# gallilmaimon/DISSC

Hardware: AMD Instinct MI355X
Metric: audio-sec/sec (RTF) HiFi-GAN resynth, 10s x32 batch (higher is better)
Workload: dtype f32

## Files before the change

dissc_amd/_lib.py:

```python
import ctypes
import os

import torch

_HERE = os.path.dirname(os.path.abspath(__file__))
_LIB_NAME = "libdissc_hip.so"


def library_path():
    return os.environ.get("DISSC_HIP_LIB") or os.path.join(_HERE, _LIB_NAME)


class DisscError(RuntimeError):
    pass


class DisscTensor(ctypes.Structure):
    _fields_ = [("name", ctypes.c_char_p), ("data", ctypes.c_void_p),
                ("shape", ctypes.c_int64 * 4), ("ndim", ctypes.c_int32)]


MAX_UPS, MAX_RK = 8, 4


class DisscGenConfig(ctypes.Structure):
    _fields_ = [("model_in_dim", ctypes.c_int32), ("upsample_initial_channel", ctypes.c_int32),
                ("num_upsamples", ctypes.c_int32), ("upsample_rates", ctypes.c_int32 * MAX_UPS),
                ("upsample_kernel_sizes", ctypes.c_int32 * MAX_UPS), ("num_kernels", ctypes.c_int32),
                ("resblock_kernel_sizes", ctypes.c_int32 * MAX_RK),
                ("resblock_dilations", (ctypes.c_int32 * 3) * MAX_RK),
                ("num_embeddings", ctypes.c_int32), ("embedding_dim", ctypes.c_int32),
                ("num_speakers", ctypes.c_int32), ("has_f0", ctypes.c_int32), ("has_spkr", ctypes.c_int32)]


class DisscConvLaunch(ctypes.Structure):
    _fields_ = [(n, ctypes.c_int32) for n in ("family", "cfg", "bm", "bn", "rows", "p0", "np", "ntap", "pad_left")]


class DisscBf3Info(ctypes.Structure):
    _fields_ = [(n, ctypes.c_int32) for n in ("bm", "bn", "small_grid", "tile", "cols", "h4", "pad")]


class DisscWino8Plan(ctypes.Structure):
    _fields_ = [(n, ctypes.c_int32) for n in ("mi", "ni", "wps", "r", "ns", "unit", "ot", "cpr", "gx", "gy")]


class DisscWinoPlan(ctypes.Structure):
    _fields_ = [(n, ctypes.c_int32) for n in ("ns", "dilation", "cpr", "rh", "tw", "shv", "unit", "ot", "gx", "gy", "wgs", "lds_bytes")]


def _load():
    path = library_path()
    if not os.path.exists(path):
        raise DisscError(
            f"{path} not found: build the HIP library first "
            "(python -c 'import __graft_entry__ as g; g.build()').  "
            "dissc_amd has no CPU fallback.")
    L = ctypes.CDLL(path)
    vp, i32, i64p = ctypes.c_void_p, ctypes.c_int, ctypes.c_void_p
    L.dissc_last_error.restype = ctypes.c_char_p
    L.dissc_abi_version.restype = i32
    L.dissc_device_count.restype = i32
    L.dissc_device_name.argtypes = [i32, ctypes.c_char_p, ctypes.c_size_t]
    L.dissc_gen_create.argtypes = [ctypes.POINTER(DisscGenConfig), ctypes.POINTER(DisscTensor),
                                   ctypes.c_size_t, ctypes.POINTER(vp)]
    L.dissc_gen_create_ex.argtypes = [ctypes.POINTER(DisscGenConfig), ctypes.POINTER(DisscTensor),
                                      ctypes.c_size_t, i32, ctypes.POINTER(vp)]
    L.dissc_gen_destroy.argtypes = [vp]
    L.dissc_gen_destroy.restype = None
    L.dissc_gen_hop.argtypes = [vp]
    L.dissc_gen_workspace_bytes.argtypes = [vp, i32, i32]
    L.dissc_gen_workspace_bytes.restype = ctypes.c_size_t
    L.dissc_gen_flops.argtypes = [vp, ctypes.c_int64]
    L.dissc_gen_flops.restype = ctypes.c_double
    L.dissc_gen_flops_executed.argtypes = [vp, ctypes.c_int64]
    L.dissc_gen_flops_executed.restype = ctypes.c_double
    L.dissc_gen_forward.argtypes = [vp, i64p, vp, i64p, vp, i32, i32, vp, vp, ctypes.c_size_t, vp]
# ... 136 lines not shown
```

dissc_amd/csrc/common.h:

```cpp
#pragma once
#include <hip/hip_runtime.h>
#include <stdint.h>
#include <stdio.h>

#include <atomic>
#include <functional>
#include <mutex>
#include <string>
#include <vector>

#include "../../include/dissc_hip.h"

#ifndef DISSC_EXPERIMENTAL
#define DISSC_EXPERIMENTAL 0
#endif

namespace dissc {

void set_error(const char* fmt, ...);

#define DISSC_OPTION_LIST_DEFAULT(X) \
  X(multistream, 1, "multistream") \
  X(pair_dma, 1, "pair_dma") \
  X(precision, 0, "precision") \
  X(enc_precision, 0, "enc_precision") \
  X(use_mfma32, 1, "mfma32") \
  X(ragged_enum, 1, "ragged_enum") \
  X(lin128, 1, "lin128") \
  X(conv2s128, 1, "conv2s128") \
  X(xcd_order, 11, "xcd_order") \
  X(xcd_mg, 0, "xcd_mg") \
  X(small_grid, 1, "small_grid") \
  X(kernel_dbg, 0, "kernel_dbg") \
  X(wino_sv, 1, "wino_sv") \
  X(wino8_c64_wide, 3, "wino8_c64_wide") \
  X(wino8_mask, 0450770550, "wino8_mask") \
  X(wino8_r4_mask, 0770770010, "wino8_r4_mask") \
  X(wino8_r4, 1, "wino8_r4") \
  X(wino8, 1, "wino8") \
  X(wino, 1, "wino") \
  X(hubert_split, 1, "hubert_split") \
  X(pair_max_c, 32, "pair_max_c") \
  X(pair_f23, 3, "pair_f23") \
  X(pair_tc6, 3, "pair_tc6") \
  X(pair_f23_c64, 1, "pair_f23_c64") \
  X(pair_tc6_c64, 1, "pair_tc6_c64")
#define DISSC_OPTION_LIST_EXPERIMENTAL(X) \
  X(graphs, 0, "graphs") \
  X(graph_frames, 2048, "graph_frames") \
  X(enc_tc, 0, "enc_tc") \
  X(s2tc_xmode, 0, "s2tc_xmode") \
  X(pair_wino, 0, "pair_wino") \
  X(pairw_chv, 2, "pairw_chv")
#if DISSC_EXPERIMENTAL
#define DISSC_OPTION_LIST(X) DISSC_OPTION_LIST_DEFAULT(X) DISSC_OPTION_LIST_EXPERIMENTAL(X)
#else
#define DISSC_OPTION_LIST(X) DISSC_OPTION_LIST_DEFAULT(X)
#endif
struct Options {
#define DISSC_OPT_FIELD(f, d, k) int f = d;
  DISSC_OPTION_LIST(DISSC_OPT_FIELD)
#undef DISSC_OPT_FIELD
#if !DISSC_EXPERIMENTAL
#define DISSC_OPT_CONST(f, d, k) static constexpr int f = d;
  DISSC_OPTION_LIST_EXPERIMENTAL(DISSC_OPT_CONST)
#undef DISSC_OPT_CONST
#endif
  int cfg_for_bm[5] = {6, 5, 7, 1, 0};
  int cfg32_for_bm[4] = {3, 2, 1, 0};
// ... 163 lines not shown
int conv32_cfg_bn(int cfg);
void conv32_set_cfg(int bm_class, int cfg);
void pack_conv_weights32(const float* w, int Cout, int Cin, int KS, std::vector<float>& packed,
                         int& Mpad, int& nchunk, int groups);
void pack_conv_weights_bf3(const float* w, int Cout, int Cin, int KS, std::vector<float>& packed,
                           int& Mpad, int& nchunk);
int launch_conv_bf3(const ConvArgs& a, int B, int Lmax_out, hipStream_t stream);
int conv_bf3_tile_bn(int M);
struct ConvBf3Plan { int tile, BM, BN, small; };
int conv_bf3_plan(int M, int KS, int dil, int groups, int B, int Lmax_out, ConvBf3Plan& p);
bool enc_bf3_supported(int Cout, int Cin, int KS, int dil, int groups, int stride, int pad_left);
int launch_enc_bf3(const ConvArgs& a, int B, int Lmax_out, int stride, hipStream_t stream);

void pack_conv_weights(const float* w, int Cout, int Cin, int KS, std::vector<float>& packed,
                       int& Mpad, int& nchunk, int groups = 1);
void convT_phase_weights(const float* w, int Cin, int Cout, int k, int s, int p0, int np, int dlo,
                         int ntap, std::vector<float>& wc);

struct DevConv {
  float* wpack = nullptr;
  float* wpack2 = nullptr;
  float* bias = nullptr;
  float* scale = nullptr;
  float* shift = nullptr;
  int CIN = 0, M = 0, KS = 0, dil = 1, nchunk = 0, up = 1;
  int groups = 1, Mpad = 0, stride = 1, pad_left = -1;
  int up_np = 1, up_p0 = 0;
  int act = 0;
  int m32 = 0;
  int prec = 0;
  double macs_per_t = 0;
  int wino = 0;
  int wr = 3;
};
struct Batch {
  const int32_t* lengths = nullptr;
  int len_default = 0, len_mul = 1, B = 0, Lmax = 0;
  const int32_t* lengths_out = nullptr;
  int olen_default = -1;
};
inline Batch batch_of(const int32_t* lengths, int len_mul, int B, int Lmax) {
  Batch bt;
  bt.lengths = lengths; bt.len_default = bt.Lmax = Lmax; bt.len_mul = len_mul; bt.B = B;
  return bt;
}
struct EpiSpec {
  int epi = EPI_STORE;
  const float* res = nullptr;
  float* acc = nullptr;
  float mrf_div = 1.f, out_slope = 0.f;
};
inline EpiSpec epi_of(int epi, const float* res = nullptr, float* acc = nullptr, float mrf_div = 1.f) {
  EpiSpec ep;
  ep.epi = epi; ep.res = res; ep.acc = acc; ep.mrf_div = mrf_div;
  return ep;
}
int upload(const std::vector<float>& h, float** d);
int pack_thread_count();
int run_pack_tasks(const std::vector<std::function<int()>>& tasks, int nthr, const Options& opt, int prec);
int conv_m32_rule(int Mg, int groups);
void conv_geometry(DevConv& dc, int Cout, int Cin, int KS, int dil, int groups, int stride, int pad_left);
struct ConvTGroup { int p0, np, dlo, ntap; };
void convT_groups(int Cout, int k, int s, std::vector<ConvTGroup>& out);
int conv_launch_cfg32(const DevConv& dc, int B, int Lmax_out);
int conv_launch_info(const DevConv& dc, int B, int Lmax_out, int* family, int* cfg, int* bm, int* bn);
int make_conv(const float* w, const float* bias, int Cout, int Cin, int KS, int dil, DevConv& dc,
              int groups = 1, int stride = 1, int pad_left = -1);
int make_convT(const float* w, const float* bias, int Cin, int Cout, int k, int s,
               std::vector<DevConv>& groups);
int set_affine(DevConv& dc, const float* scale, const float* shift, int n);
void free_conv(DevConv& dc);
int run_conv(const DevConv& dc, const float* x, float* out, const Batch& bt, const EpiSpec& ep, int C_x, int ldx, int ldo,
             float slope, hipStream_t stream, int dma_in = 0);

bool wino_supported(int Cout, int Cin, int KS, int dil);
int make_wino(const float* w, const float* bias, int C, int KS, int dil, DevConv& dc);
double wino_executed_macs_per_t(int C, int KS);
int run_wino(const DevConv& dc, const float* x, float* out, const Batch& bt, const EpiSpec& ep, int ldx, int ldo, float slope,
             hipStream_t stream);
struct WinoPlan { int inst, NS, dil, CPR, RH, TW, SHV, unit, OT, gx, gy, wgs, lds_bytes; };
int wino_plan(int C, int KS, int dil, int B, int Lmax, WinoPlan& p);

bool wino8_supported(int Cout, int Cin, int KS, int dil);
bool wino8_r4_supported(int C, int KS, int dil);
int make_wino8(const float* w, const float* bias, int C, int KS, int dil, DevConv& dc, int R = 3);
double wino8_executed_macs_per_t(int C, int KS, int R);
int run_wino8(const DevConv& dc, const float* x, float* out, const Batch& bt, const EpiSpec& ep, int ldx, int ldo, float slope,
              hipStream_t stream);
struct Wino8Plan { int inst, R, NS, MI, NI, WPS, unit, OT, CPR, gx, gy; };
int wino8_plan(int C, int KS, int dil, int R, int B, int Lmax, Wino8Plan& p);

struct DevPairW {
  float* w1 = nullptr;
  float* w2 = nullptr;
  float* b1 = nullptr;
  float* b2 = nullptr;
  int C = 0, KS = 0, dil = 1;
  int form = 0;
};
bool pair_f23_supported(int C, int KS, int dil);
bool pair_tc6_supported(int C, int KS, int dil);
bool pairw43_built();
int pack_pairw43(const float* w, int C, int KS, float** dev);
int launch_pairw43(const DevPairW& pw, const float* x, float* out, const Batch& bt, const EpiSpec& ep, int ld, float slope,
                   hipStream_t stream);
bool pairw_supported(int C, int KS, int dil);
bool pair_form_supported(int form, int C, int KS, int dil);
int pair_reg_tile(int form, int C, int KS, int dil);
int make_pairw(const float* w1, const float* b1, const float* w2, const float* b2, int C, int KS, int dil, int form, DevPairW& pw);
void free_pairw(DevPairW& pw);
int launch_respair_wino(const DevPairW& pw, const float* x, float* out, const Batch& bt, const EpiSpec& ep, int ld, float slope,
                        hipStream_t stream);

bool respair_supported(int C, int KS, int dil);
int launch_respair(const DevConv& c1, const DevConv& c2, const float* x, float* out, const Batch& bt, const EpiSpec& ep, int ld,
                   float slope, hipStream_t stream);

bool resblock_bf3_supported(int C, int KS, const int* dil);
void pack_resblock_bf3(int C, int KS, const float* const* w6, std::vector<float>& packed);
struct Bf3Block { int C, KS; const int* dil; const float *wpack, *bias; };
int launch_resblock_bf3(const Bf3Block& blk, const float* x, const Batch& bt, const EpiSpec& ep, int ld, float slope, int m0, int m1,
                        hipStream_t stream);
// ... 30 lines not shown
```

dissc_amd/csrc/conv_wino8.hip:

```cpp
#include <string.h>

#include <type_traits>

#include "common.h"
#include "conv_epilogue32.h"
#include "wino_common.h"

namespace dissc {


struct Wino8Args {
  const float* x;
  const float* wpack;
  const float* bias;
  const float* res;
  float* out;
  float* acc;
  const int32_t* lengths;
  int len_default, len_mul;
  int C, nchunk, pad;
  int ldx, ldo;
  long long x_bstride, o_bstride;
  float slope, mrf_div;
  int epi;
  int dbg;
  int gx, gy, B;
};

static const double kW8Pt[7] = {0.0, 1.0, -1.0, 2.0, -2.0, 0.5, -0.5};
static const double kW8Scale[7] = {-1.0, -2.0 / 9.0, -2.0 / 9.0, 1.0 / 90.0, 1.0 / 90.0, 32.0 / 45.0, 32.0 / 45.0};
static double w8_g(int p, int i, int R) {
  if (p == 7) return i == R - 1 ? 1.0 : 0.0;
  double v = kW8Scale[p];
  for (int e = 0; e < i; ++e) v *= kW8Pt[p];
  return v;
}

template <int P>
__device__ __forceinline__ float w8_bt(float r0, float r1, float r2, float r3, float r4, float r5, float r6, float r7) {
  if constexpr (P == 0) return fmaf(5.25f, r2 - r4, r6 - r0);
  if constexpr (P == 1) return fmaf(-4.25f, r3 + r4, (r1 + r2) + (r5 + r6));
  if constexpr (P == 2) return fmaf(4.25f, r3 - r4, (r2 - r1) + (r6 - r5));
  if constexpr (P == 3) return fmaf(0.5f, r1, fmaf(0.25f, r2, fmaf(-2.5f, r3, fmaf(-1.25f, r4, fmaf(2.f, r5, r6)))));
  if constexpr (P == 4) return fmaf(-0.5f, r1, fmaf(0.25f, r2, fmaf(2.5f, r3, fmaf(-1.25f, r4, fmaf(-2.f, r5, r6)))));
  if constexpr (P == 5) return fmaf(2.f, r1, fmaf(4.f, r2, fmaf(-2.5f, r3, fmaf(-5.f, r4, fmaf(0.5f, r5, r6)))));
  if constexpr (P == 6) return fmaf(-2.f, r1, fmaf(4.f, r2, fmaf(2.5f, r3, fmaf(-5.f, r4, fmaf(-0.5f, r5, r6)))));
  if constexpr (P == 7) return fmaf(5.25f, r3 - r5, r7 - r1);
  return 0.f;
}

constexpr int w8_rup(int n, int m) { return (n + m - 1) / m * m; }

constexpr int w8_row_len(int D, int NTU, int need, int MO) {
// ... 53 lines not shown
template <int NS, int DIL, int MI, int NI, int WPS = 2, int R = 3>
__global__ void __launch_bounds__(512, (NI == 1 ? 2 : WPS)) conv_wino8_kernel(const Wino8Args a) {
  using G = Wino8Geo<NS, DIL, MI, NI, WPS, R>;
  constexpr bool LAT = G::LAT;
  constexpr int NTH = G::NTH, D = G::D, W = G::W, NCOL = G::NCOL, OT = G::OT, NV = G::NV, RL = G::RL, MO = G::MO,
                CHF = G::CHF, CPR = G::CPR, XV = G::XV, YS = G::YS, OFF = G::OFF, RPP = G::RPP, CG = G::CG;
  extern __shared__ __attribute__((aligned(16))) float lds[];
  float* const vbuf = lds + G::WIN_FLOATS;

  const int per = 8 / a.gy;
  const int xcd = blockIdx.x & 7, kq = blockIdx.x >> 3;
  const int mt = xcd / per;
  const int lin = (xcd - mt * per) + per * kq;
  if (lin >= a.gx * a.B) return;
  const int tid = threadIdx.x;
  const int lane = tid & 63;
  int b, len = a.len_default, t0;
  if (a.lengths == nullptr) {
    b = lin / a.gx;
    t0 = (lin - b * a.gx) * OT;
    if (t0 >= len) return;
  } else {
    int tile;
    if (!ragged_tile<OT>(lin, a.B, [&](int i) { return a.lengths[i] * a.len_mul; }, b, tile, len)) return;
    t0 = tile * OT;
  }
  const int p = __builtin_amdgcn_readfirstlane(tid >> 6);
  const int l31 = lane & 31, h = lane >> 5;
  const int o = t0 - a.pad;
  const int tb = o & ~3;
  const int sh = o - tb;
  const float slope = a.slope;
  const float* xb = a.x + (size_t)b * a.x_bstride;
  const int nround = a.C / CPR;

  const int r0 = tid / NV, v0 = tid - r0 * NV;
  constexpr int dr = NTH / NV, dv = NTH - dr * NV;
  constexpr int SV = (CPR * NV + NTH - 1) / NTH;
  f32x4 sv[SV];
  auto stage_load = [&](int rd) __attribute__((always_inline)) {
    int r = r0, v = v0;
#pragma unroll
    for (int i = 0; i < SV; ++i) {
      int ci = rd * CPR + (r < CPR ? r : CPR - 1);
      ci = ci < a.C ? ci : a.C - 1;
      int t = tb + 4 * v;
      t = t < 0 ? 0 : (t > a.ldx - 4 ? a.ldx - 4 : t);
      sv[i] = *reinterpret_cast<const f32x4*>(xb + (size_t)ci * a.ldx + t);
      v += dv;
      r += dr;
      if (v >= NV) { v -= NV; ++r; }
    }
  };
  auto stage_store = [&](float* raw) __attribute__((always_inline)) {
    int r = r0, v = v0;
#pragma unroll
    for (int i = 0; i < SV; ++i) {
      if (r < CPR) {
        const int t = tb + 4 * v;
        const f32x4 val = sv[i];
        float* rowp = raw + r * CHF;
#pragma unroll
        for (int e = 0; e < 4; ++e) {
          const bool ok = (t + e) >= 0 && (t + e) < len;
          const int xs = 4 * v + e - sh + OFF * D;
          rowp[(xs % D) * RL + xs / D] = ok ? lrelu(val[e], slope) : 0.f;
        }
// ... 59 lines not shown
  int voff[NI];
#pragma unroll
  for (int ni = 0; ni < NI; ++ni) {
    int col = ni * 32 + l31;
    col = col < NCOL ? col : NCOL - 1;
    voff[ni] = (col / D) * W + (col % D) + h * XV;
  }
  f32x16 acc[MI][NI];
#pragma unroll
  for (int mi = 0; mi < MI; ++mi)
#pragma unroll
    for (int ni = 0; ni < NI; ++ni)
#pragma unroll
      for (int e = 0; e < 16; ++e) acc[mi][ni][e] = 0.f;

  const int nsub = a.C / 32;
  const int nblk = a.nchunk * NS * 2;
  f32x4 av[MI], avn[MI];
#ifndef DISSC_WINO8_BUF
#define DISSC_WINO8_BUF 1
#endif
#if DISSC_WINO8_BUF
  const __amdgpu_buffer_rsrc_t wrs = wave_rsrc(reinterpret_cast<const f32x4*>(a.wpack) + ((size_t)p * nsub + mt * MI) * nblk * 64,
                                               (unsigned)(MI * nblk) * 1024u);
  const unsigned lane16 = lane * 16u;
  auto a_load = [&](int mi, int bl) __attribute__((always_inline)) { return rsrc_load16(wrs, lane16, (unsigned)(mi * nblk + bl) * 1024u); };
#else
  const f32x4* wp[MI];
#pragma unroll
  for (int mi = 0; mi < MI; ++mi)
    wp[mi] = reinterpret_cast<const f32x4*>(a.wpack) + ((size_t)p * nsub + mt * MI + mi) * nblk * 64 + lane;
  auto a_load = [&](int mi, int bl) __attribute__((always_inline)) { return wp[mi][(size_t)bl * 64]; };
#endif
  if constexpr (!LAT) {
#pragma unroll
    for (int mi = 0; mi < MI; ++mi) av[mi] = a_load(mi, 0);
  }
  stage_load(0);
  stage_store(lds);
  if (nround > 1) stage_load(1);
  __syncthreads();

  if constexpr (LAT) {
    constexpr int SCR = CPR / 8;
    static_assert(SCR == 2, "latency form: two sub-chunks per round");
    const int tcol = l31 < NCOL ? l31 : NCOL - 1;
    const int toffl = (tcol % D) * RL + MO * (tcol / D) + OFF + 4 * h * CHF;
    const int e0l = (tcol / D) * W + tcol % D + 4 * h * XV;
    const bool ok1l = tcol % D + D < W;
    const int e1l = ok1l ? e0l + D : e0l;
    float* const vt[2] = {vbuf + p * (8 * XV), vbuf + 8 * 8 * XV + p * (8 * XV)};
    float q[4][9];
    auto tr_read = [&](const float* raw8) __attribute__((always_inline)) {
#pragma unroll
      for (int ii = 0; ii < 4; ++ii) {
        const float* rw = raw8 + ii * CHF + toffl;
        if constexpr (MO % 2 == 0) {
#pragma unroll
          for (int e = 0; e < 8; e += 2) {
            const f32x2a t = *reinterpret_cast<const f32x2a*>(rw + e);
            q[ii][e] = t[0];
            q[ii][e + 1] = t[1];
          }
        } else {
#pragma unroll
          for (int e = 0; e < 8; ++e) q[ii][e] = rw[e];
        }
        q[ii][8] = NS > 1 ? rw[8] : 0.f;
      }
    };
    auto tr_piece = [&](auto pc, float* vdst, int ii) __attribute__((always_inline)) {
      constexpr int P = decltype(pc)::value;
      const float v0 = w8_bt<P>(q[ii][0], q[ii][1], q[ii][2], q[ii][3], q[ii][4], q[ii][5], q[ii][6], q[ii][7]);
      vdst[ii * XV + e0l] = v0;
      if constexpr (NS > 1) {
        const float v1 = w8_bt<P>(q[ii][1], q[ii][2], q[ii][3], q[ii][4], q[ii][5], q[ii][6], q[ii][7], q[ii][8]);
        vdst[ii * XV + e1l] = ok1l ? v1 : v0;
      }
    };
    f32x4 aq[SCR][NS][MI];
#pragma unroll
    for (int sc = 0; sc < SCR; ++sc)
#pragma unroll
      for (int j = 0; j < NS; ++j)
#pragma unroll
        for (int mi = 0; mi < MI; ++mi) aq[sc][j][mi] = a_load(mi, sc * NS + j);
    int blk = 0;
    auto slot = [&](auto pc, auto scc, const float* raw_next) __attribute__((always_inline)) {
      constexpr int SC = decltype(scc)::value;
      tr_read(raw_next);
      const float* bj = vt[SC & 1] + voff[0];
#pragma unroll
      for (int j = 0; j < NS; ++j, ++blk) {
        float bk[4];
#pragma unroll
        for (int s = 0; s < 4; ++s) bk[s] = bj[s * 2 * XV + j * DIL];
#pragma unroll
        for (int s = 0; s < 4; ++s)
#pragma unroll
          for (int mi = 0; mi < MI; ++mi)
            acc[mi][0] = __builtin_amdgcn_mfma_f32_32x32x2f32(aq[SC][j][mi][s], bk[s], acc[mi][0], 0, 0, 0);
        const int bn = blk + SCR * NS < nblk ? blk + SCR * NS : nblk - 1;
#pragma unroll
        for (int mi = 0; mi < MI; ++mi) aq[SC][j][mi] = a_load(mi, bn);
      }
#pragma unroll
      for (int ii = 0; ii < 4; ++ii) tr_piece(pc, vt[(SC + 1) & 1], ii);
    };
    auto body = [&](auto pc) __attribute__((always_inline)) {
      tr_read(lds);
#pragma unroll
      for (int ii = 0; ii < 4; ++ii) tr_piece(pc, vt[0], ii);
      for (int rd = 0; rd < nround; ++rd) {
        const float* raw = lds + (rd & 1) * (CPR * CHF);
        float* rawn = lds + ((rd + 1) & 1) * (CPR * CHF);
        if (rd + 1 < nround) stage_store(rawn);
        if (rd + 2 < nround) stage_load(rd + 2);
        slot(pc, std::integral_constant<int, 0>{}, raw + 8 * CHF);
        __syncthreads();
        slot(pc, std::integral_constant<int, 1>{}, rawn);
      }
    };
    switch (p) {
      case 0: body(std::integral_constant<int, 0>{}); break;
      case 1: body(std::integral_constant<int, 1>{}); break;
      case 2: body(std::integral_constant<int, 2>{}); break;
      case 3: body(std::integral_constant<int, 3>{}); break;
      case 4: body(std::integral_constant<int, 4>{}); break;
      case 5: body(std::integral_constant<int, 5>{}); break;
      case 6: body(std::integral_constant<int, 6>{}); break;
      default: body(std::integral_constant<int, 7>{}); break;
    }
    __syncthreads();
  }

  int blk = 0;
  auto run_taps = [&]() __attribute__((always_inline)) {
    if (a.dbg & 2) {
      blk += NS;
      return;
    }
    const float* bj[NI];
#pragma unroll
    for (int ni = 0; ni < NI; ++ni) bj[ni] = vp + voff[ni];
#pragma unroll
    for (int j = 0; j < NS; ++j, ++blk) {
      const int bn = (blk + 1 < nblk) ? blk + 1 : nblk - 1;
#pragma unroll
      for (int mi = 0; mi < MI; ++mi) avn[mi] = a_load(mi, bn);
      float bk[4][NI];
#pragma unroll
      for (int s = 0; s < 4; ++s)
#pragma unroll
        for (int ni = 0; ni < NI; ++ni) bk[s][ni] = bj[ni][s * 2 * XV + j * DIL];
      __builtin_amdgcn_sched_barrier(0);
#pragma unroll
      for (int s = 0; s < 4; ++s)
#pragma unroll
        for (int mi = 0; mi < MI; ++mi)
#pragma unroll
          for (int ni = 0; ni < NI; ++ni)
            acc[mi][ni] = __builtin_amdgcn_mfma_f32_32x32x2f32(av[mi][s], bk[s][ni], acc[mi][ni], 0, 0, 0);
      __builtin_amdgcn_sched_barrier(0);
#pragma unroll
      for (int mi = 0; mi < MI; ++mi) av[mi] = avn[mi];
    }
  };

  for (int rd = 0; rd < (LAT ? 0 : nround); ++rd) {
    const float* raw = lds + (rd & 1) * (CPR * CHF);
    if (rd + 1 < nround) stage_store(lds + ((rd + 1) & 1) * (CPR * CHF));
    if (rd + 2 < nround) stage_load(rd + 2);
#pragma unroll
    for (int sc = 0; sc < CPR / 8; ++sc) {
      transform8(raw + (sc * 8) * CHF);
      run_taps();
    }
    __syncthreads();
  }

  float* const yb = lds;
  float* const ot = lds + G::Y_FLOATS;
  if (a.dbg & 4) {
    if (acc[0][0][0] == 123.f) a.out[0] = 1.f;
    return;
  }
  const int epi = a.epi;
  const size_t ob = (size_t)b * a.o_bstride;
  constexpr int OS = G::OS;
  constexpr bool AL = OT % 4 == 0;
  constexpr int QPR = AL ? OT / 4 : (OT + 3) / 4 + 1;
  constexpr int NQ = RPP * QPR, NIT = (NQ + NTH - 1) / NTH;
  const int qsh = AL ? 0 : (t0 & 3);
  const int tend = (t0 + OT < len) ? t0 + OT : len;
  constexpr int NCI = RPP * NCOL, NCT = (NCI + NTH - 1) / NTH;
  constexpr int PS = RPP * YS;
  constexpr int NPASS = 32 * MI / RPP;
#pragma unroll
  for (int ps = 0; ps < NPASS; ++ps) {
    const int mi = ps * RPP / 32;
    const int sp = (ps * RPP % 32) / 16;
    f32x4 pres[NIT], pacc[NIT];
    const bool rmw = epi != EPI_STORE && epi != EPI_RES && epi != EPI_MRF_SET;
    if (epi != EPI_STORE) {
#pragma unroll
      for (int it = 0; it < NIT; ++it) {
        const int idx = tid + it * NTH;
        const int row = idx / QPR, qi = idx - row * QPR;
        const int n0 = t0 - qsh + 4 * qi;
        if (idx < NQ && n0 >= t0 && n0 + 4 <= tend) {
          const size_t ixp = ob + (size_t)(mt * (32 * MI) + ps * RPP + row) * a.ldo + n0;
          pres[it] = *reinterpret_cast<const f32x4*>(a.res + ixp);
          if (rmw) pacc[it] = *reinterpret_cast<const f32x4*>(a.acc + ixp);
        }
      }
    }
    if (ps > 0) __syncthreads();
#pragma unroll
    for (int ni = 0; ni < NI; ++ni)
#pragma unroll
      for (int r = 0; r < 16; ++r) {
        if constexpr (RPP == 32) {
          yb[(p * 32 + (r & 3) + 8 * (r >> 2) + 4 * h) * YS + ni * 32 + l31] = acc[mi][ni][r];
        } else {
          if ((r >> 3) == sp) yb[(p * 16 + (r & 3) + 8 * ((r >> 2) & 1) + 4 * h) * YS + ni * 32 + l31] = acc[mi][ni][r];
        }
      }
    __syncthreads();
#pragma unroll
    for (int it = 0; it < NCT; ++it) {
      const int idx = tid + it * NTH;
      if (idx >= NCI) continue;
      const int row = idx / NCOL, c = idx - row * NCOL;
      const int tau = c / D, rho = c - tau * D;
      const float* yc = yb + row * YS + c;
      const float y0 = yc[0], y1 = yc[PS], y2 = yc[2 * PS], y3 = yc[3 * PS], y4 = yc[4 * PS], y5 = yc[5 * PS], y6 = yc[6 * PS],
                  y7 = yc[7 * PS];
      const float s12 = y1 + y2, d12 = y1 - y2, s34 = y3 + y4, d34 = y3 - y4, s56 = y5 + y6, d56 = y5 - y6;
      float* op = ot + row * OS + MO * D * tau + rho;
      op[0] = (y0 + s12) + (s34 + s56);
      op[D] = fmaf(2.f, d34, fmaf(0.5f, d56, d12));
      op[2 * D] = fmaf(4.f, s34, fmaf(0.25f, s56, s12));
      op[3 * D] = fmaf(8.f, d34, fmaf(0.125f, d56, d12));
      if constexpr (MO == 6) {
        op[4 * D] = fmaf(16.f, s34, fmaf(0.0625f, s56, s12));
        op[5 * D] = fmaf(32.f, d34, fmaf(0.03125f, d56, d12)) + y7;
      } else {
        op[4 * D] = fmaf(16.f, s34, fmaf(0.0625f, s56, s12)) + y7;
      }
    }
    __syncthreads();
#pragma unroll
    for (int it = 0; it < NIT; ++it) {
      const int idx = tid + it * NTH;
      if (idx >= NQ) continue;
      const int row = idx / QPR, qi = idx - row * QPR;
      const int n0 = t0 - qsh + 4 * qi;
      const int lo = n0 > t0 ? n0 : t0, hi = n0 + 4 < tend ? n0 + 4 : tend;
      if (hi <= lo) continue;
      const int grow = mt * (32 * MI) + ps * RPP + row;
      const float bz = a.bias[grow];
      f32x4 v;
      if constexpr (AL) {
        v = *reinterpret_cast<const f32x4*>(ot + row * OS + 4 * qi);
      } else {
        const float* src = ot + row * OS + (4 * qi - qsh);
#pragma unroll
        for (int e = 0; e < 4; ++e) v[e] = (4 * qi - qsh + e >= 0) ? src[e] : 0.f;
      }
      v[0] += bz; v[1] += bz; v[2] += bz; v[3] += bz;
      const size_t ix = ob + (size_t)grow * a.ldo + n0;
      if (hi - lo == 4) {
        epi_store(epi, quad_at(a.out + ix), quad_at(a.acc + ix), v, [&] { return pres[it]; }, [&] { return pacc[it]; }, a.mrf_div);
      } else {
        float rr[4], aa[4];
#pragma unroll
        for (int e = 0; e < 4; ++e) {
          const bool ok = n0 + e >= lo && n0 + e < hi;
          rr[e] = (ok && epi != EPI_STORE) ? a.res[ix + e] : 0.f;
          aa[e] = (ok && rmw) ? a.acc[ix + e] : 0.f;
        }
#pragma unroll
        for (int e = 0; e < 4; ++e) {
          if (n0 + e < lo || n0 + e >= hi) continue;
          epi_store(epi, a.out + ix + e, a.acc + ix + e, v[e], [&] { return rr[e]; }, [&] { return aa[e]; }, a.mrf_div);
        }
      }
    }
  }
}

bool wino8_supported(int Cout, int Cin, int KS, int dil) {
  if (KS == 3 && !DISSC_EXPERIMENTAL && !(Cout == 64 && dil == 1)) return false;
  return Cout == Cin && (Cout == 64 || Cout == 128 || Cout == 256 || Cout == 512) && (KS == 3 || KS == 7 || KS == 11) &&
         (dil == 1 || dil == 3 || dil == 5);
}

bool wino8_r4_supported(int C, int KS, int dil) { return wino8_supported(C, C, KS, dil) && (KS == 7 || KS == 11); }

int make_wino8(const float* w, const float* bias, int C, int KS, int dil, DevConv& dc, int R) {
  if (R != 3 && !(R == 4 && wino8_r4_supported(C, KS, dil))) {
    set_error("make_wino8: no instance with %d-tap sub-filters for C = %d, k = %d, dilation %d", R, C, KS, dil);
    return DISSC_EINVAL;
  }
  if (C % 32 != 0 || C % KC != 0) {
    set_error("make_wino8: C = %d is not a multiple of the row tile", C);
    return DISSC_EINVAL;
  }
  const int nchunk = C / KC;
  const std::vector<float> packed = pack_wino_weights(w, C, KS, 8, R, [R](int p, int i) { return w8_g(p, i, R); });
  std::vector<float> b(C, 0.f);
  if (bias) memcpy(b.data(), bias, C * sizeof(float));
  dc.CIN = C; dc.M = C; dc.KS = KS; dc.dil = dil; dc.nchunk = nchunk; dc.up = 1;
  dc.groups = 1; dc.Mpad = C; dc.stride = 1; dc.pad_left = -1; dc.m32 = 1; dc.prec = 0;
  dc.macs_per_t = (double)C * C * KS;
  dc.wino = 2;
  dc.wr = R;
  int rc = upload(packed, &dc.wpack);
  if (rc) return rc;
  return upload(b, &dc.bias);
}

double wino8_executed_macs_per_t(int C, int KS, int R) { return (double)C * C * 8.0 * ((KS + R - 1) / R) / (9.0 - R); }

template <int NS, int DIL, int MI, int NI, int WPS = 2, int R = 3>
static int launch_wino8_t(const Wino8Args& a, hipStream_t stream) {
  using G = Wino8Geo<NS, DIL, MI, NI, WPS, R>;
  static DeviceOnce attr_once;
  DISSC_HIP_CHECK(attr_once.max_lds(reinterpret_cast<const void*>(&conv_wino8_kernel<NS, DIL, MI, NI, WPS, R>), 160 * 1024));
  const int per = 8 / a.gy;
  dim3 grid(8 * ((a.gx * a.B + per - 1) / per));
  hipLaunchKernelGGL((conv_wino8_kernel<NS, DIL, MI, NI, WPS, R>), grid, dim3(512), (size_t)G::LDS_FLOATS * sizeof(float), stream, a);
  DISSC_HIP_CHECK(hipGetLastError());
  return DISSC_OK;
}

struct Wino8Inst {
  int R, NS, dil, MI, NI, WPS;
  int unit, OT, CPR;
  int (*launch)(const Wino8Args&, hipStream_t);
};
#define DISSC_W8_INST(R_, NS_, D_, MI_, NI_, WPS_)                                                                   \
  {R_, NS_, D_, MI_, NI_, WPS_, Wino8Geo<NS_, D_, MI_, NI_, WPS_, R_>::MO * Wino8Geo<NS_, D_, MI_, NI_, WPS_, R_>::D, \
   Wino8Geo<NS_, D_, MI_, NI_, WPS_, R_>::OT, Wino8Geo<NS_, D_, MI_, NI_, WPS_, R_>::CPR,                             \
   &launch_wino8_t<NS_, D_, MI_, NI_, WPS_, R_>}
#define DISSC_W8_SHAPE(R_, NS_, D_)                                                                                    \
  DISSC_W8_INST(R_, NS_, D_, 1, 1, 4), DISSC_W8_INST(R_, NS_, D_, 2, 1, 4), DISSC_W8_INST(R_, NS_, D_, 2, 2, 4),       \
  DISSC_W8_INST(R_, NS_, D_, 4, 2, 2), DISSC_W8_INST(R_, NS_, D_, 2, 4, 2), DISSC_W8_INST(R_, NS_, D_, 2, 2, 2)
static const Wino8Inst kW8Inst[] = {
#if DISSC_EXPERIMENTAL
// ... 27 lines not shown
  const bool sg = opts().small_grid != 0;
  auto tiles_of = [&](int MI, int NI, int WPS, int rows) -> long long {
    const int i = w8_find(R, ns, dil, MI, NI, WPS);
    if (i < 0) return -1;
    return (long long)((Lmax + kW8Inst[i].OT - 1) / kW8Inst[i].OT) * (C / rows) * B;
  };
  int MI, NI, WPS;
  if (ns == 1 && !DISSC_EXPERIMENTAL) {
    MI = 2; NI = 2; WPS = 4;
  } else if (C >= 128) {
    const long long nwg = tiles_of(4, 2, 2, 128);
    if (sg && nwg >= 0 && nwg < 32) { MI = C / 32 > 8 ? 2 : 1; NI = 1; WPS = 4; }
    else if (sg && nwg >= 0 && nwg < 64) { MI = 2; NI = 1; WPS = 4; }
    else if (sg && nwg >= 0 && nwg < 128) { MI = 2; NI = 2; WPS = 4; }
    else { MI = 4; NI = 2; WPS = 2; }
  } else {
    const long long nwg = tiles_of(2, 2, 4, 64);
    if (sg && nwg >= 0 && nwg < 192) { MI = 2; NI = 1; WPS = 4; }
    else if (c64_mode == 1) { MI = 2; NI = 4; WPS = 2; }
    else if (c64_mode == 2) { MI = 2; NI = 2; WPS = 4; }
    else { MI = 2; NI = 2; WPS = 2; }
  }
  const int i = w8_find(R, ns, dil, MI, NI, WPS);
  if (i < 0) {
    set_error("wino8_plan: no %d x %d tile (%d waves per SIMD) for k = %d, dilation %d, %d-tap sub-filters", 32 * MI, 32 * NI, WPS, KS, dil, R);
    return DISSC_EINVAL;
  }
  const Wino8Inst& t = kW8Inst[i];
  p.inst = i;
  p.R = R; p.NS = ns; p.MI = MI; p.NI = NI; p.WPS = WPS;
  p.unit = t.unit; p.OT = t.OT; p.CPR = t.CPR;
  p.gx = (Lmax + t.OT - 1) / t.OT;
  p.gy = C / (32 * MI);
  if (p.gy < 1 || 8 % p.gy != 0) {
    set_error("wino8_plan: %d row tiles do not divide the 8 XCDs", p.gy);
    return DISSC_EINVAL;
  }
  if (C % t.CPR != 0) {
    set_error("wino8_plan: %d channels are not a multiple of the %d a round stages", C, t.CPR);
    return DISSC_EINVAL;
  }
  return DISSC_OK;
}

int run_wino8(const DevConv& dc, const float* x, float* out, const Batch& bt, const EpiSpec& ep, int ldx, int ldo, float slope,
              hipStream_t stream) {
  Wino8Args a;
  a.x = x; a.wpack = dc.wpack; a.bias = dc.bias; a.res = ep.res; a.out = out; a.acc = ep.acc;
  a.lengths = bt.lengths; a.len_default = bt.len_default; a.len_mul = bt.len_mul;
  a.C = dc.M; a.nchunk = dc.nchunk; a.pad = (dc.KS - 1) * dc.dil / 2;
  a.ldx = ldx; a.ldo = ldo;
  a.x_bstride = (long long)dc.M * ldx; a.o_bstride = (long long)dc.M * ldo;
  a.slope = slope; a.mrf_div = ep.mrf_div; a.epi = ep.epi; a.dbg = opts().kernel_dbg;
  a.gx = a.gy = a.B = 0;
  if (ldx < 4 || ldx % 4 || ldo % 4 || misaligned16(x) || misaligned16(out) || misaligned16(ep.res) || misaligned16(ep.acc)) {
    set_error("run_wino8: rows must be 16-byte aligned (ldx %d, ldo %d: multiples of 4 floats, ldx >= 4)", ldx, ldo);
    return DISSC_EINVAL;
  }
  Wino8Plan p;
  const int rc = wino8_plan(dc.M, dc.KS, dc.dil, dc.wr == 4 ? 4 : 3, bt.B, bt.Lmax, p);
  if (rc) return rc;
  a.gx = p.gx; a.gy = p.gy; a.B = bt.B;
  return kW8Inst[p.inst].launch(a, stream);
}

}
```

dissc_amd/csrc/diag.hip:

```cpp
#include <stdlib.h>

#include <algorithm>
#include <vector>

#include "gen_plan.h"

using namespace dissc;

namespace {

struct DiagScope {
  DevConv c1, c2;
  DevPairW pw;
  DevS2tc tc;
  std::vector<float*> bufs;
  hipEvent_t e0 = nullptr, e1 = nullptr;
  hipError_t alloc(float** p, size_t n) {
    const hipError_t e = hipMalloc((void**)p, n * sizeof(float));
    if (e == hipSuccess) bufs.push_back(*p);
    return e;
  }
  hipError_t events() {
    const hipError_t e = hipEventCreate(&e0);
    return e != hipSuccess ? e : hipEventCreate(&e1);
// ... 239 lines not shown
      (up == 1 && k % 2 != 1) || (up > 1 && ((k - up) % 2 != 0 || k < up || dilation != 1))) {
    set_error("dissc_conv_info: bad argument");
    return DISSC_EINVAL;
  }
  std::vector<ConvTGroup> plan;
  if (up > 1) convT_groups(Cout, k, up, plan);
  else plan.push_back(ConvTGroup{0, 1, 0, k});
  int n = 0;
  for (const ConvTGroup& g : plan) {
    DevConv dc;
    conv_geometry(dc, Cout * g.np, Cin, g.ntap, up > 1 ? 1 : dilation, 1, 1, up > 1 ? -g.dlo : -1);
    int family, cfg, bm, bn;
    const int rc = conv_launch_info(dc, B, Lmax_out, &family, &cfg, &bm, &bn);
    if (rc) return rc;
    if (n < max_out) {
      DisscConvLaunch& o = out[n];
      o.family = family; o.cfg = cfg; o.bm = bm; o.bn = bn; o.rows = dc.M;
      o.p0 = g.p0; o.np = g.np; o.ntap = g.ntap;
      o.pad_left = dc.pad_left >= 0 ? dc.pad_left : ((dc.KS - 1) * dc.dil) / 2;
    }
    ++n;
  }
  if (n_out) *n_out = n;
  return DISSC_OK;
}

int dissc_wino8_info(int C, int k, int dilation, int R, int B, int Lmax, DisscWino8Plan* out) {
  Wino8Plan p;
  const int rc = wino8_plan(C, k, dilation, R, B, Lmax, p);
  if (rc) return rc;
  if (out) {
    out->mi = p.MI; out->ni = p.NI; out->wps = p.WPS; out->r = p.R; out->ns = p.NS;
    out->unit = p.unit; out->ot = p.OT; out->cpr = p.CPR; out->gx = p.gx; out->gy = p.gy;
  }
  return DISSC_OK;
}

int dissc_wino_info(int C, int k, int dilation, int B, int Lmax, DisscWinoPlan* out) {
  WinoPlan p;
  const int rc = wino_plan(C, k, dilation, B, Lmax, p);
  if (rc) return rc;
  if (out) {
    out->ns = p.NS; out->dilation = p.dil; out->cpr = p.CPR; out->rh = p.RH; out->tw = p.TW; out->shv = p.SHV;
    out->unit = p.unit; out->ot = p.OT; out->gx = p.gx; out->gy = p.gy; out->wgs = p.wgs; out->lds_bytes = p.lds_bytes;
  }
  return DISSC_OK;
}

int dissc_pair_bench(int B, int C, int k, int dilation, int L, int epi, int iters, int mode, float* ms_out) {
  if (!ms_out || B <= 0 || L <= 0 || iters <= 0 || epi < EPI_RES || epi > EPI_MRF_DIV) {
    set_error("dissc_pair_bench: bad argument");
    return DISSC_EINVAL;
  }
  std::vector<float> w1((size_t)C * C * k), w2((size_t)C * C * k), bias(C, 0.1f);
  Lcg rnd;
  rnd.fill(w1, 0.05f);
  rnd.fill(w2, 0.05f);
  DiagScope ds;
  int rc = pair_make(mode, w1.data(), bias.data(), w2.data(), bias.data(), C, k, dilation, ds);
  if (rc) return rc;
  const int ld = (L + 3) / 4 * 4;
  const size_t n = (size_t)B * C * ld;
  float *x = nullptr, *y = nullptr, *t = nullptr, *a = nullptr;
  std::vector<float> hx(n);
  rnd.fill(hx, 2.f);
  if (ds.alloc(&x, n) != hipSuccess || ds.alloc(&y, n) != hipSuccess || ds.alloc(&t, n) != hipSuccess ||
// ... 128 lines not shown
```

dissc_amd/csrc/gen_plan.hip:

```cpp
#include "gen_plan.h"

namespace dissc {

constexpr int WINO_MIN_C = 64;
constexpr int WINO_C64_KMIN = 3;
static bool wino_wanted(int C, int KS) {
  if (!opts().wino || C < WINO_MIN_C) return false;
  if (C < 128 && KS < WINO_C64_KMIN) return false;
  return wino_supported(C, C, KS, 1);
}

static int w8_shape_bit(int C, int KS, int dil) {
  const int cls = C >= 256 ? 2 : C >= 128 ? 1 : 0;
  return 9 * cls + 3 * (KS == 11 ? 2 : KS == 7 ? 1 : 0) + (dil == 1 ? 0 : dil == 3 ? 1 : 2);
}
ConvForm td_conv_form(int C, int KS, int dil) {
  if (!opts().wino8 || !wino8_supported(C, C, KS, dil) || !((opts().wino8_mask >> w8_shape_bit(C, KS, dil)) & 1))
    return ConvForm::f43;
  const bool r4 = opts().wino8_r4 && wino8_r4_supported(C, KS, dil) && ((opts().wino8_r4_mask >> w8_shape_bit(C, KS, dil)) & 1);
  return r4 ? ConvForm::f54 : ConvForm::f63;
}

int pair_reg_form(int C, int KS, int dil) {
  if (C == 64) {
    if (opts().pair_f23 == 0) return 0;
    if (KS == 3) return opts().pair_f23_c64 && pair_f23_supported(C, KS, dil) ? 1 : 0;
    const int bit = KS == 7 ? 1 : KS == 11 ? 2 : 0;
    return (opts().pair_tc6_c64 & bit) && pair_tc6_supported(C, KS, dil) ? 2 : 0;
  }
  if (C != 16 && C != 32) return 0;
  const int stage = C == 32 ? 1 : 2;
  if (KS == 3) return pair_f23_supported(C, KS, dil) && (opts().pair_f23 & (stage << 2)) ? 1 : 0;
  if (!(opts().pair_f23 & stage)) return 0;
  const int tc6_bit = (C == 32 ? 1 : 4) << (KS == 11 ? 1 : 0);
  if ((KS == 7 || KS == 11) && (opts().pair_tc6 & tc6_bit) && pair_tc6_supported(C, KS, dil)) return 2;
  return pair_f23_supported(C, KS, dil) ? 1 : 0;
}
static bool pairw_wanted(int C, int KS, int dil) {
  if (pair_reg_form(C, KS, dil)) return true;
  if (!opts().pair_wino || !pairw_supported(C, KS, dil)) return false;
  if (opts().pair_wino >= 2) return true;
  if (C == 32) return KS == 11 && dil <= 3;
  return C == 64 && KS == 3 && dil == 1;
}

ChainPlan plan_chain(int C, int KS, const int* dil, int prec) {
  ChainPlan cp;
// ... 55 lines not shown
```

include/dissc_hip.h:

```cpp
#ifndef DISSC_HIP_H
#define DISSC_HIP_H

#include <stddef.h>
#include <stdint.h>

#ifdef __cplusplus
extern "C" {
#endif

#define DISSC_OK 0
#define DISSC_EINVAL (-1)
#define DISSC_ENOMEM (-2)
#define DISSC_EHIP (-3)
#define DISSC_ENOTFOUND (-4)
#define DISSC_ENOTSUP (-5)
#define DISSC_ECOMM (-6)

typedef struct {
  const char* name;
  const float* data;
  int64_t shape[4];
  int32_t ndim;
} DisscTensor;

// ... 47 lines not shown
int dissc_conv_transpose1d_prec(const float* x, const float* w_host, const float* bias_host, float* y,
                                const int32_t* lengths, int B, int Cin, int Cout, int k, int stride,
                                int ldx, int ldo, int Lmax, float in_slope, int prec, void* stream);

int dissc_conv1d_s2(const float* x, const float* w_host, const float* bias_host, float* y, const int32_t* lengths_in, int B,
                    int Cin, int Cout, int k, int ldx, int ldo, int Lmax_in, int act, int form, void* stream);
int dissc_conv1d_s2_prec(const float* x, const float* w_host, const float* bias_host, float* y, const int32_t* lengths_in, int B,
                         int Cin, int Cout, int k, int ldx, int ldo, int Lmax_in, int act, int prec, void* stream);
int dissc_linear_prec(const float* x, const float* w_host, const float* bias_host, const float* res, float* y,
                      const int32_t* lengths, int B, int Cin, int Cout, int ld, int Tmax, int act, int prec, void* stream);
int dissc_conv_s2_bench(int B, int C, int L, int form, int iters, float* ms_out);

int dissc_set_option(const char* key, int value);
int dissc_get_option(const char* key, int* value);

int dissc_conv_bench(int B, int Cin, int Cout, int k, int dilation, int L, int epi, int iters,
                     int flags, float* ms_out);

int dissc_respair1d(const float* x, const float* w1_host, const float* b1_host, const float* w2_host, const float* b2_host,
                    float* y, float* acc, const int32_t* lengths, int B, int C, int k, int dilation, int ld, int Lmax,
                    float slope, int epi, float mrf_div, int mode, void* stream);
int dissc_pair_bench(int B, int C, int k, int dilation, int L, int epi, int iters, int mode, float* ms_out);
int dissc_pair_info(int C, int k, int dilation, int* form_out, int* tile_out);
typedef struct {
  int32_t family, cfg, bm, bn, rows;
  int32_t p0, np, ntap, pad_left;
} DisscConvLaunch;
int dissc_conv_info(int Cin, int Cout, int k, int dilation, int up, int B, int Lmax_out, DisscConvLaunch* out, int max_out,
                    int* n_out);

typedef struct {
  int32_t mi, ni, wps, r, ns;
  int32_t unit, ot, cpr, gx, gy;
} DisscWino8Plan;
int dissc_wino8_info(int C, int k, int dilation, int R, int B, int Lmax, DisscWino8Plan* out);

typedef struct {
  int32_t ns, dilation, cpr, rh, tw, shv;
  int32_t unit, ot, gx, gy, wgs, lds_bytes;
} DisscWinoPlan;
int dissc_wino_info(int C, int k, int dilation, int B, int Lmax, DisscWinoPlan* out);

int dissc_resblock1d_bf3(const float* x, const float* const* w6_host, const float* const* b6_host, float* acc,
                         const int32_t* lengths, int B, int C, int k, const int32_t* dil3, int ld, int Lmax, float slope,
                         int epi, float mrf_div, int m0, int m1, void* stream);
typedef struct {
  int32_t bm, bn, small_grid, tile;
  int32_t cols, h4, pad;
} DisscBf3Info;
int dissc_bf3_info(int Cout, int Cin, int k, int dilation, int B, int Lmax, const int32_t* dil3, int m0, int m1,
                   DisscBf3Info* out);

typedef struct dissc_pred* dissc_pred_t;
int dissc_pred_create(int kind, const DisscTensor* weights, size_t n_weights, dissc_pred_t* out);
void dissc_pred_destroy(dissc_pred_t p);
size_t dissc_pred_workspace_bytes(dissc_pred_t p, int B, int Lmax);
int dissc_len_set_norm(dissc_pred_t p, float mean, float std);
int dissc_len_forward(dissc_pred_t p, const int64_t* seq, const int64_t* spk, const int32_t* lengths,
                      int B, int Lmax, float* out, int ldo, void* workspace, size_t workspace_bytes,
                      void* stream);
int dissc_pitch_forward(dissc_pred_t p, const int64_t* seq, const int64_t* spk,
                        const int32_t* lengths, int B, int Tmax, int norm, const float* id2mean,
                        const float* id2std, int n_stats, float* out, int ldo, void* workspace,
                        size_t workspace_bytes, void* stream);
int dissc_pitch_stats(const double* f0, const int64_t* offsets, int n_speakers, double* mean_out,
                      double* std_out, int64_t* count_out, void* stream);
// ... 203 lines not shown
```

Baseline: 10320.

## Split wino8 channel reduction into sequential accumulation blocks for selected shapes

Adds an option to split the Winograd F(6,3)-style conv's input-channel reduction into several sequential kernel launches, each covering a contiguous range of channel chunks. Later blocks read the partial output back as a residual and skip the bias, and the real epilogue is applied only on the final block. It is enabled by a shape mask for large-channel, kernel-11 layers, aiming to shrink per-launch working set or pipeline length. It costs extra launches plus an additional round trip of the output tensor through memory.

```diff
diff --git a/dissc_amd/_lib.py b/dissc_amd/_lib.py
--- a/dissc_amd/_lib.py
+++ b/dissc_amd/_lib.py
@@ -42,7 +42,7 @@
 
 
 class DisscWino8Plan(ctypes.Structure):
-    _fields_ = [(n, ctypes.c_int32) for n in ("mi", "ni", "wps", "r", "ns", "unit", "ot", "cpr", "gx", "gy")]
+    _fields_ = [(n, ctypes.c_int32) for n in ("mi", "ni", "wps", "r", "ns", "unit", "ot", "cpr", "gx", "gy", "kblocks")]
 
 
 class DisscWinoPlan(ctypes.Structure):
diff --git a/dissc_amd/csrc/common.h b/dissc_amd/csrc/common.h
--- a/dissc_amd/csrc/common.h
+++ b/dissc_amd/csrc/common.h
@@ -35,6 +35,8 @@
   X(wino_sv, 1, "wino_sv") \
   X(wino8_c64_wide, 3, "wino8_c64_wide") \
   X(wino8_mask, 0450770550, "wino8_mask") \
+  X(wino8_kblock, 0300000000, "wino8_kblock") \
+  X(wino8_kblocks, 2, "wino8_kblocks") \
   X(wino8_r4_mask, 0770770010, "wino8_r4_mask") \
   X(wino8_r4, 1, "wino8_r4") \
   X(wino8, 1, "wino8") \
@@ -264,6 +266,7 @@
   double macs_per_t = 0;
   int wino = 0;
   int wr = 3;
+  int kblocks = 0;
 };
 struct Batch {
   const int32_t* lengths = nullptr;
@@ -319,7 +322,8 @@
 double wino8_executed_macs_per_t(int C, int KS, int R);
 int run_wino8(const DevConv& dc, const float* x, float* out, const Batch& bt, const EpiSpec& ep, int ldx, int ldo, float slope,
               hipStream_t stream);
-struct Wino8Plan { int inst, R, NS, MI, NI, WPS, unit, OT, CPR, gx, gy; };
+struct Wino8Plan { int inst, R, NS, MI, NI, WPS, unit, OT, CPR, gx, gy, kblocks; };
+int wino8_kblocks_of(int C, int KS, int dil);
 int wino8_plan(int C, int KS, int dil, int R, int B, int Lmax, Wino8Plan& p);
 
 struct DevPairW {
diff --git a/dissc_amd/csrc/conv_wino8.hip b/dissc_amd/csrc/conv_wino8.hip
--- a/dissc_amd/csrc/conv_wino8.hip
+++ b/dissc_amd/csrc/conv_wino8.hip
@@ -19,6 +19,7 @@
   const int32_t* lengths;
   int len_default, len_mul;
   int C, nchunk, pad;
+  int kc0, kblock;
   int ldx, ldo;
   long long x_bstride, o_bstride;
   float slope, mrf_div;
@@ -138,7 +139,9 @@
   const int sh = o - tb;
   const float slope = a.slope;
   const float* xb = a.x + (size_t)b * a.x_bstride;
-  const int nround = a.C / CPR;
+  const int rb = a.kc0 * KC / CPR;
+  const int nround = a.kblock ? rb + a.kblock * KC / CPR : a.C / CPR;
+  const bool first = a.kc0 == 0, final = nround * CPR >= a.C;
 
   const int r0 = tid / NV, v0 = tid - r0 * NV;
   constexpr int dr = NTH / NV, dv = NTH - dr * NV;
@@ -264,13 +267,14 @@
     wp[mi] = reinterpret_cast<const f32x4*>(a.wpack) + ((size_t)p * nsub + mt * MI + mi) * nblk * 64 + lane;
   auto a_load = [&](int mi, int bl) __attribute__((always_inline)) { return wp[mi][(size_t)bl * 64]; };
 #endif
+  const int blk0 = rb * (CPR / 8) * NS;
   if constexpr (!LAT) {
 #pragma unroll
-    for (int mi = 0; mi < MI; ++mi) av[mi] = a_load(mi, 0);
-  }
-  stage_load(0);
-  stage_store(lds);
-  if (nround > 1) stage_load(1);
+    for (int mi = 0; mi < MI; ++mi) av[mi] = a_load(mi, blk0);
+  }
+  stage_load(rb);
+  stage_store(lds + (rb & 1) * (CPR * CHF));
+  if (rb + 1 < nround) stage_load(rb + 1);
   __syncthreads();
 
   if constexpr (LAT) {
@@ -316,8 +320,8 @@
 #pragma unroll
       for (int j = 0; j < NS; ++j)
 #pragma unroll
-        for (int mi = 0; mi < MI; ++mi) aq[sc][j][mi] = a_load(mi, sc * NS + j);
-    int blk = 0;
+        for (int mi = 0; mi < MI; ++mi) aq[sc][j][mi] = a_load(mi, blk0 + sc * NS + j);
+    int blk = blk0;
     auto slot = [&](auto pc, auto scc, const float* raw_next) __attribute__((always_inline)) {
       constexpr int SC = decltype(scc)::value;
       tr_read(raw_next);
@@ -340,10 +344,10 @@
       for (int ii = 0; ii < 4; ++ii) tr_piece(pc, vt[(SC + 1) & 1], ii);
     };
     auto body = [&](auto pc) __attribute__((always_inline)) {
-      tr_read(lds);
+      tr_read(lds + (rb & 1) * (CPR * CHF));
 #pragma unroll
       for (int ii = 0; ii < 4; ++ii) tr_piece(pc, vt[0], ii);
-      for (int rd = 0; rd < nround; ++rd) {
+      for (int rd = rb; rd < nround; ++rd) {
         const float* raw = lds + (rd & 1) * (CPR * CHF);
         float* rawn = lds + ((rd + 1) & 1) * (CPR * CHF);
         if (rd + 1 < nround) stage_store(rawn);
@@ -366,7 +370,7 @@
     __syncthreads();
   }
 
-  int blk = 0;
+  int blk = blk0;
   auto run_taps = [&]() __attribute__((always_inline)) {
     if (a.dbg & 2) {
       blk += NS;
@@ -399,7 +403,7 @@
     }
   };
 
-  for (int rd = 0; rd < (LAT ? 0 : nround); ++rd) {
+  for (int rd = rb; rd < (LAT ? rb : nround); ++rd) {
     const float* raw = lds + (rd & 1) * (CPR * CHF);
     if (rd + 1 < nround) stage_store(lds + ((rd + 1) & 1) * (CPR * CHF));
     if (rd + 2 < nround) stage_load(rd + 2);
@@ -417,7 +421,8 @@
     if (acc[0][0][0] == 123.f) a.out[0] = 1.f;
     return;
   }
-  const int epi = a.epi;
+  const int epi = final ? ((first || a.epi != EPI_STORE) ? a.epi : EPI_RES) : ((first && a.epi == EPI_STORE) ? EPI_STORE : EPI_RES);
+  const float* const rsrc = first ? a.res : a.out;
   const size_t ob = (size_t)b * a.o_bstride;
   constexpr int OS = G::OS;
   constexpr bool AL = OT % 4 == 0;
@@ -442,7 +447,7 @@
         const int n0 = t0 - qsh + 4 * qi;
         if (idx < NQ && n0 >= t0 && n0 + 4 <= tend) {
           const size_t ixp = ob + (size_t)(mt * (32 * MI) + ps * RPP + row) * a.ldo + n0;
-          pres[it] = *reinterpret_cast<const f32x4*>(a.res + ixp);
+          pres[it] = *reinterpret_cast<const f32x4*>(rsrc + ixp);
           if (rmw) pacc[it] = *reinterpret_cast<const f32x4*>(a.acc + ixp);
         }
       }
@@ -491,7 +496,7 @@
       const int lo = n0 > t0 ? n0 : t0, hi = n0 + 4 < tend ? n0 + 4 : tend;
       if (hi <= lo) continue;
       const int grow = mt * (32 * MI) + ps * RPP + row;
-      const float bz = a.bias[grow];
+      const float bz = first ? a.bias[grow] : 0.f;
       f32x4 v;
       if constexpr (AL) {
         v = *reinterpret_cast<const f32x4*>(ot + row * OS + 4 * qi);
@@ -509,7 +514,7 @@
 #pragma unroll
         for (int e = 0; e < 4; ++e) {
           const bool ok = n0 + e >= lo && n0 + e < hi;
-          rr[e] = (ok && epi != EPI_STORE) ? a.res[ix + e] : 0.f;
+          rr[e] = (ok && epi != EPI_STORE) ? rsrc[ix + e] : 0.f;
           aa[e] = (ok && rmw) ? a.acc[ix + e] : 0.f;
         }
 #pragma unroll
@@ -540,6 +545,11 @@
     return DISSC_EINVAL;
   }
   const int nchunk = C / KC;
+  const int kblocks = wino8_kblocks_of(C, KS, dil);
+  if (kblocks && nchunk % kblocks != 0) {
+    set_error("make_wino8: %d accumulation blocks (\"wino8_kblocks\") do not divide the %d channel chunks of C = %d", kblocks, nchunk, C);
+    return DISSC_EINVAL;
+  }
   const std::vector<float> packed = pack_wino_weights(w, C, KS, 8, R, [R](int p, int i) { return w8_g(p, i, R); });
   std::vector<float> b(C, 0.f);
   if (bias) memcpy(b.data(), bias, C * sizeof(float));
@@ -548,6 +558,7 @@
   dc.macs_per_t = (double)C * C * KS;
   dc.wino = 2;
   dc.wr = R;
+  dc.kblocks = kblocks;
   int rc = upload(packed, &dc.wpack);
   if (rc) return rc;
   return upload(b, &dc.bias);
@@ -641,6 +652,7 @@
   p.unit = t.unit; p.OT = t.OT; p.CPR = t.CPR;
   p.gx = (Lmax + t.OT - 1) / t.OT;
   p.gy = C / (32 * MI);
+  p.kblocks = wino8_kblocks_of(C, KS, dil);
   if (p.gy < 1 || 8 % p.gy != 0) {
     set_error("wino8_plan: %d row tiles do not divide the 8 XCDs", p.gy);
     return DISSC_EINVAL;
@@ -670,7 +682,14 @@
   const int rc = wino8_plan(dc.M, dc.KS, dc.dil, dc.wr == 4 ? 4 : 3, bt.B, bt.Lmax, p);
   if (rc) return rc;
   a.gx = p.gx; a.gy = p.gy; a.B = bt.B;
-  return kW8Inst[p.inst].launch(a, stream);
-}
-
-}
+  const int nb = dc.kblocks > 1 ? dc.kblocks : 1;
+  for (int i = 0; i < nb; ++i) {
+    a.kblock = nb > 1 ? dc.nchunk / nb : 0;
+    a.kc0 = i * a.kblock;
+    const int lrc = kW8Inst[p.inst].launch(a, stream);
+    if (lrc) return lrc;
+  }
+  return DISSC_OK;
+}
+
+}
diff --git a/dissc_amd/csrc/diag.hip b/dissc_amd/csrc/diag.hip
--- a/dissc_amd/csrc/diag.hip
+++ b/dissc_amd/csrc/diag.hip
@@ -295,6 +295,7 @@
   if (out) {
     out->mi = p.MI; out->ni = p.NI; out->wps = p.WPS; out->r = p.R; out->ns = p.NS;
     out->unit = p.unit; out->ot = p.OT; out->cpr = p.CPR; out->gx = p.gx; out->gy = p.gy;
+    out->kblocks = p.kblocks;
   }
   return DISSC_OK;
 }
diff --git a/dissc_amd/csrc/gen_plan.hip b/dissc_amd/csrc/gen_plan.hip
--- a/dissc_amd/csrc/gen_plan.hip
+++ b/dissc_amd/csrc/gen_plan.hip
@@ -13,6 +13,10 @@
 static int w8_shape_bit(int C, int KS, int dil) {
   const int cls = C >= 256 ? 2 : C >= 128 ? 1 : 0;
   return 9 * cls + 3 * (KS == 11 ? 2 : KS == 7 ? 1 : 0) + (dil == 1 ? 0 : dil == 3 ? 1 : 2);
+}
+int wino8_kblocks_of(int C, int KS, int dil) {
+  const int n = opts().wino8_kblocks;
+  return n > 1 && ((opts().wino8_kblock >> w8_shape_bit(C, KS, dil)) & 1) ? n : 0;
 }
 ConvForm td_conv_form(int C, int KS, int dil) {
   if (!opts().wino8 || !wino8_supported(C, C, KS, dil) || !((opts().wino8_mask >> w8_shape_bit(C, KS, dil)) & 1))
diff --git a/include/dissc_hip.h b/include/dissc_hip.h
--- a/include/dissc_hip.h
+++ b/include/dissc_hip.h
@@ -103,6 +103,7 @@
 typedef struct {
   int32_t mi, ni, wps, r, ns;
   int32_t unit, ot, cpr, gx, gy;
+  int32_t kblocks;
 } DisscWino8Plan;
 int dissc_wino8_info(int C, int k, int dilation, int R, int B, int Lmax, DisscWino8Plan* out);
 
```

Result: no change. 10310 (-0.1%).
